# amcpherson/remixt

Measured on AMD Instinct MI355X. Metric: EM iterations/sec (50k seg x 165 states), higher is better.
Workload: dtype f64

## Files before the change

remixt_amd/csrc/rmx_kernels.h:

```cpp
#pragma once
#include "rmx_device.h"
#include "rmx_host.h"
#define SEGL 32
#define SEG_PER_BLOCK (256 / SEGL)
#define TRIAL_SEGL 16
#define RMX_CLUSTER_SPINS (1u << 22)
#define FBK_WKN 128
#define NM_MAX_SAMPLE 1024
#define TRIAL_SEG_PER_BLOCK (256 / TRIAL_SEGL)


__device__ __forceinline__ void state_tables_body(const Dev &d, int cls, int r, const RestartParams &rp) {
    __shared__ unsigned agg_sh;
    if (threadIdx.x == 0) agg_sh = 0u;
    __syncthreads();
    unsigned agg = 0u;
    for (int s = threadIdx.x; s < d.S; s += blockDim.x) {
        const int8_t *cn = d.cn + ((size_t)cls * d.S + s) * d.M * 2;
        const int8_t *tot = d.tot + ((size_t)cls * d.S + s) * d.M;
        double minor = 0., total = 0.;
        for (int m = 0; m < d.M; m++) {
            minor += rp.h[m] * (double)cn[m * 2 + 0];
            total += rp.h[m] * (double)tot[m];
        }
        const unsigned sf = d.sflags[(size_t)cls * d.S + s];
        const bool hdel = sf & 1u, loh = sf & 2u;
        unsigned fl = 0;
        if (!d.nc && hdel) fl |= ST_HDEL_NB;
        double p;
        if (hdel) p = 0.;
        else {
            if (total <= 0.) { fl |= ST_E_TD; p = 0.5; }
            else p = minor / total;
        }
        double M0, M1;
        if (!d.nc && loh) {
            if (p == 0.) p = rp.p[RMX_P_BETABIN_LOH_P];
            else if (p == 1.) p = 1. - rp.p[RMX_P_BETABIN_LOH_P];
            else if (!(fl & ST_E_TD)) fl |= ST_E_LOH;
            M0 = rp.p[RMX_P_BETABIN_LOH_M_0]; M1 = rp.p[RMX_P_BETABIN_LOH_M_1];
            fl |= ST_LOH_M | ST_GZ_ALLELE;
        } else {
            M0 = rp.p[RMX_P_BETABIN_M_0]; M1 = rp.p[RMX_P_BETABIN_M_1];
        }
        if (p <= 0. || (1 - p) <= 0.) fl |= ST_E_BADP;
        const size_t base = ((size_t)r * d.C + cls);
        const size_t si = base * d.SP + s;
        d.stD[si] = total;
        d.stLogD[si] = total > 0. ? log(total) : 0.;
        d.stP[si] = p;
        d.stM[(base * 2 + 0) * d.SP + s] = M0;
        d.stM[(base * 2 + 1) * d.SP + s] = M1;
        const bool ok = !(fl & (ST_E_BADP | ST_E_TD | ST_E_LOH));
        d.stLg[(base * 4 + 0) * d.SP + s] = ok ? lgamma_pos(M0 * p) : 0.;
        d.stLg[(base * 4 + 1) * d.SP + s] = ok ? lgamma_pos(M0 * (1 - p)) : 0.;
        d.stLg[(base * 4 + 2) * d.SP + s] = ok ? lgamma_pos(M1 * p) : 0.;
        d.stLg[(base * 4 + 3) * d.SP + s] = ok ? lgamma_pos(M1 * (1 - p)) : 0.;
        d.stFlags[si] = fl;
        agg |= ((fl & ST_E_TD) ? 1u : 0u) | ((fl & ST_E_LOH) ? 2u : 0u) | (((fl & ST_E_BADP) && !(fl & (ST_E_TD | ST_E_LOH))) ? 4u : 0u);
    }
    if (agg) atomicOr(&agg_sh, agg);
    __syncthreads();
    if (threadIdx.x == 0) d.stFlagsAgg[(size_t)r * d.C + cls] = agg_sh;
}
__global__ void k_state_tables(Dev d, int r0) {
    const int cls = blockIdx.x, r = r0 + blockIdx.y;
    const RestartParams rp = d.rp[r];
    state_tables_body(d, cls, r, rp);
}
__global__ void k_state_tables_one(Dev d, int r, RestartParams rp) {
    if (blockIdx.x == 0 && threadIdx.x == 0) d.rp[r] = rp;
    state_tables_body(d, blockIdx.x, r, rp);
}

__device__ __forceinline__ double seg_const_value(const RestartParams &rp, double x, double y0, double ys, int i) {
    if (i < 4) {
        const double rr = i == 0 ? rp.p[RMX_P_NEGBIN_R_0] : (i == 1 ? rp.p[RMX_P_NEGBIN_HDEL_R_0] : (i == 2 ? rp.p[RMX_P_NEGBIN_R_1] : rp.p[RMX_P_NEGBIN_HDEL_R_1]));
        return lgamma_pos(x + rr) - lgamma_pos(x + 1) - lgamma_pos(rr);
    }
    const double MM = i == 4 ? rp.p[RMX_P_BETABIN_M_0] : (i == 5 ? rp.p[RMX_P_BETABIN_LOH_M_0] : (i == 6 ? rp.p[RMX_P_BETABIN_M_1] : rp.p[RMX_P_BETABIN_LOH_M_1]));
    return (lgamma_pos(ys + 1) - lgamma_pos(y0 + 1) - lgamma_pos(ys - y0 + 1)) - lgamma_pos(ys + MM) + lgamma_pos(MM);
}
__global__ void k_seg_const(Dev d, int r0) {
    const int n = blockIdx.x * blockDim.x + threadIdx.x, r = r0 + blockIdx.y;
    if (n >= d.N) return;
    const RestartParams &rp = d.rp[r];
    const double x = d.x[n], y0 = d.y[2 * (size_t)n], y1 = d.y[2 * (size_t)n + 1], ys = y0 + y1;
    double *sc = d.segc + (size_t)r * 8 * d.N + n;
#pragma unroll
    for (int i = 0; i < 8; i++) sc[(size_t)i * d.N] = seg_const_value(rp, x, y0, ys, i);
}

__global__ void k_framelogprob(Dev d, int r0, int G) {
    const int r = r0 + blockIdx.y;
    const int rows = 256 / G;
    const int n = blockIdx.x * rows + threadIdx.x / G, gl = threadIdx.x % G;
    if (n >= d.N) return;
    const RestartParams &rp = d.rp[r];
    SegCtx sc; load_seg(d, r, n, sc);
    const int cls = d.seg_class[n];
    const double qt0 = d.qt[((size_t)r * d.N + n) * 2], qt1 = d.qt[((size_t)r * d.N + n) * 2 + 1];
    const double qa0 = d.qa[((size_t)r * d.N + n) * 2], qa1 = d.qa[((size_t)r * d.N + n) * 2 + 1];
    const double qs0 = d.qs[((size_t)r * d.N + n) * 2], qs1 = d.qs[((size_t)r * d.N + n) * 2 + 1];
    double *frow = d.f + rs_off(d, r, n);
    unsigned err = 0;
    double vmax = -INFINITY;
    for (int s = gl; s < d.S; s += G) {
        double LT[2], LA[4];
        cell_ll(d, rp, sc, r, cls, s, LT, LA, err);
        double f = 0.;
        f += qt0 * LT[0]; f += qt1 * LT[1];
        f += qa0 * qs0 * LA[0]; f += qa0 * qs1 * LA[1]; f += qa1 * qs0 * LA[2]; f += qa1 * qs1 * LA[3];
        f += cell_prior(d, rp, sc, cls, s);
        if (f != f) err |= RMX_ERR_NAN_F;
        frow[s] = f;
        vmax = f > vmax ? f : vmax;
    }
    vmax = group_max(vmax, G);
    if (gl == 0) d.fmax[(size_t)r * d.N + n] = vmax;
    double *erow = d.fe + rs_off(d, r, n);
    for (int s = gl; s < d.SP; s += G) erow[s] = s < d.S ? exp_fast(frow[s] - vmax) : 0.;
    if (err) atomicOr(&d.err[r], err);
}

#define FB_NBUF 3

struct FbLaunch { int P, NT, BLK, SPAD; };

struct FbArgs {
    int S, SP, M, D, C, N, NBE, cn_max, P, BLK, SPAD, r0, amat_lds, pad_;
    double pen;
    const int32_t *chain_start, *chain_end, *tclass, *brk_slot, *chain_list, *chain_tc, *chain_cls, *be_cls;
    const double *fe, *Wf, *Wb, *pe_lt;
    const int8_t *af, *ab, *tot;
    double *fa, *fb, *mrow;
    uint32_t *err;
    unsigned long long *dbg;
};

typedef const __attribute__((address_space(1))) void *gptr_t;
typedef __attribute__((address_space(3))) void *lptr_t;

#define FB_BARRIER() asm volatile("s_waitcnt lgkmcnt(0)\n\ts_barrier" ::: "memory")

__device__ __forceinline__ void glds16(const void *gsrc, unsigned lds_dst_uniform) {
    unsigned keep;
    asm volatile("s_mov_b32 %0, m0\n\ts_mov_b32 m0, %2\n\ts_nop 0\n\tglobal_load_lds_dwordx4 %1, off\n\ts_mov_b32 m0, %0"
                 : "=&s"(keep) : "v"(gsrc), "s"(lds_dst_uniform) : "memory");
}
__device__ __forceinline__ void glds4(const void *gsrc, unsigned lds_dst_uniform) {
    unsigned keep;
    asm volatile("s_mov_b32 %0, m0\n\ts_mov_b32 m0, %2\n\ts_nop 0\n\tglobal_load_lds_dword %1, off\n\ts_mov_b32 m0, %0"
                 : "=&s"(keep) : "v"(gsrc), "s"(lds_dst_uniform) : "memory");
}
__device__ __forceinline__ void gload8(double &dst, const double *src) {
    asm volatile("global_load_dwordx2 %0, %1, off" : "=v"(dst) : "v"(src) : "memory");
}
__device__ __forceinline__ void gwait8(double &v) { asm volatile("s_waitcnt vmcnt(0)" : "+v"(v) :: "memory"); }
__device__ __forceinline__ void gwait8_after(double &v, double &after) { asm volatile("s_waitcnt vmcnt(0)" : "+v"(v), "+v"(after) :: "memory"); }
__device__ __forceinline__ void gstore8(double *dst, double v) {
    asm volatile("global_store_dwordx2 %0, %1, off\n\ts_nop 1" ::"v"(dst), "v"(v) : "memory");
}
__device__ __forceinline__ unsigned lds_addr(const void *p) { return (unsigned)(size_t)(lptr_t)p; }

#ifdef RMX_FB_STAMPS
#define FB_STAMP(i_) { unsigned long long t_; asm volatile("s_memtime %0\n\ts_waitcnt lgkmcnt(0)" : "=s"(t_) :: "memory"); stamp_acc[i_] += t_ - stamp_last; stamp_last = t_; }
#else
#define FB_STAMP(i_)
#endif
template <int NTMAX>
__global__ __launch_bounds__(NTMAX) void k_fb(FbArgs a) {
    extern __shared__ __align__(16) unsigned char smem_raw[];
    const int chain = a.chain_list[blockIdx.x], r = a.r0 + blockIdx.y, dir = blockIdx.z;
    const int S = a.S, M = a.M, D = a.D, SP = a.SP;
    const int n0 = a.chain_start[chain], n1 = a.chain_end[chain], len = n1 - n0 + 1;
    const int t = threadIdx.x, NT = blockDim.x;
    const int PP = a.P;
    const int p = t / S, o = t - p * S;
    const bool act = p < PP;
    const bool post = t < S;
    const int QPT = (S + PP - 1) / PP;
    const int SPAD = a.SPAD, BLK = a.BLK;
    const int MDP = (M * D + 1) & ~1;
    double *ebuf = (double *)smem_raw;
    double *vec = ebuf + (size_t)FB_NBUF * BLK * SP;
    double *part = vec + 2 * SPAD;
    double *red = part + (size_t)PP * SP;
    double *pel = red + 4;
    double *wa = pel + MDP;
    int *meta = (int *)(wa + 128);
    int8_t *totl = (int8_t *)(meta + FB_NBUF * 2 * 64);
    for (int i = t; i < a.C * S * M; i += NT) totl[i] = a.tot[i];
    for (int i = t; i < 2 * SPAD; i += NT) vec[i] = 0.;
    for (int i = t; i < 128; i += NT) wa[i] = exp(-a.pen * (double)i);
    for (int i = t; i < FB_NBUF * 2 * 64; i += NT) meta[i] = -1;
    unsigned long long *red64 = reinterpret_cast<unsigned long long *>(red);
    if (t < 4) red64[t] = 0ull;

    const size_t rbase = (size_t)r * a.N;
    const double *febase = a.fe + rbase * SP;
    double *outb = (dir == 0 ? a.fa : a.fb) + rbase * SP;
    double *mrow = a.mrow + rbase;
    const double *Wmat = dir == 0 ? a.Wf : a.Wb;

    __syncthreads();

#define ROW(k) (dir == 0 ? n0 + (k) : n1 - (k))
    const int nblk = (len + BLK - 1) / BLK;
    const int elems = BLK * SP / 2;
    const int wave_base = (t >> 6) << 6;
#define FB_ISSUE(b_)                                                                                                   \
    {                                                                                                                  \
        const int slot_ = (b_) % FB_NBUF;                                                                              \
        const int rs_ = dir == 0 ? n0 + (b_) * BLK : n1 - (b_) * BLK - (BLK - 1);                                      \
        for (int i0 = 0; i0 < elems; i0 += NT) {                                                                       \
            const int idx = i0 + t;                                                                                    \
            const int row_ = rs_ + (idx * 2) / SP;                                                                     \
            const unsigned dst_ = __builtin_amdgcn_readfirstlane(lds_addr(ebuf + (size_t)slot_ * BLK * SP + (size_t)(i0 + wave_base) * 2)); \
            if (idx < elems && row_ >= n0 && row_ <= n1) glds16(febase + (size_t)rs_ * SP + (size_t)idx * 2, dst_);   \
        }                                                                                                              \
        if (t < 64) {                                                                                                  \
            const int tn_ = (dir == 0 ? n0 + (b_) * BLK - 1 : n1 - (b_) * BLK - (BLK - 1)) + t;                        \
            const unsigned d0_ = __builtin_amdgcn_readfirstlane(lds_addr(meta + (slot_ * 2 + 0) * 64));                 \
            const unsigned d1_ = __builtin_amdgcn_readfirstlane(lds_addr(meta + (slot_ * 2 + 1) * 64));                 \
            if (t < BLK && tn_ >= n0 && tn_ < n1) { glds4(a.tclass + tn_, d0_); glds4(a.brk_slot + tn_, d1_); }        \
        }                                                                                                              \
    }

    FB_ISSUE(0)
    if (nblk > 1) FB_ISSUE(1)
    asm volatile("s_waitcnt vmcnt(0)" ::: "memory");
    if (nblk > 2) FB_ISSUE(2)
    FB_BARRIER();

    const int rstep = dir == 0 ? SP : -SP;
    double *outp = outb + (size_t)ROW(0) * SP + o;
    double *mptr = mrow + ROW(0);
    const int npw = (S + 63) >> 6;
    {
        double e0 = 0.;
        if (post) { e0 = ebuf[(size_t)(dir == 0 ? 0 : BLK - 1) * SP + o]; vec[o] = e0; gstore8(outp, (dir == 0) ? e0 : 1.0); }
        if ((t >> 6) < npw) {
            const double wm = wave_max_nonneg(e0);
            if ((t & 63) == 0) lds_max_u64(&red64[0], (unsigned long long)__double_as_longlong(wm));
        }
    }
    FB_BARRIER();

    int b = 0, kk = 0, slot = 0;
    int cur = 0, nxt = 1;
    int rc = 0;
    if (a.dbg && t == 0 && blockIdx.x == 0 && blockIdx.y == 0 && blockIdx.z == 0) { a.dbg[0] = clock64(); a.dbg[1] = wall_clock64(); a.dbg[4] = len; }
#ifdef RMX_FB_STAMPS
    unsigned long long stamp_acc[6] = {0, 0, 0, 0, 0, 0}, stamp_last;
    asm volatile("s_memtime %0\n\ts_waitcnt lgkmcnt(0)" : "=s"(stamp_last) :: "memory");
#endif
    for (int k = 1; k < len; k++) {
        FB_STAMP(0)
        if (++kk == BLK) { kk = 0; b++; slot = slot + 1 == FB_NBUF ? 0 : slot + 1; }
        const int kidx = dir == 0 ? kk : BLK - 1 - kk;
        const double *vc = vec + cur * SPAD;
        const int bs = meta[(slot * 2 + 1) * 64 + kidx];
        const int rn = rc + 1 == 3 ? 0 : rc + 1, rz = rn + 1 == 3 ? 0 : rn + 1;
        double inv = 0., e = 0.;
        if ((t >> 6) < npw) {
            double m;
            pow2_scale((unsigned)(red64[rc] >> 32), m, inv);
            if (post) e = ebuf[((size_t)slot * BLK + kidx) * SP + o];
            if (t == 0) { if (dir == 0) gstore8(mptr, m); red64[rz] = 0ull; }
        }
        FB_STAMP(1)
        double acc = 0.;
        if (bs < 0) {
            const double *Wt = Wmat + (size_t)meta[(slot * 2 + 0) * 64 + kidx] * S * S;
            if (act) for (int rr = 0; rr < QPT; rr++) { const int q = p * QPT + rr; if (q < S) acc = fma(vc[q], Wt[(size_t)q * S + o], acc); }
        } else {
            const int tc = meta[(slot * 2 + 0) * 64 + kidx];
            if (t < 64) {
                const unsigned dpe = __builtin_amdgcn_readfirstlane(lds_addr(pel));
                if (t * 2 < MDP) glds16(a.pe_lt + ((size_t)r * a.NBE + bs) * MDP + t * 2, dpe);
            }
            asm volatile("s_waitcnt vmcnt(0)" ::: "memory");
            FB_BARRIER();
            int ca, cb;
            const int8_t *at;
            ca = a.be_cls[2 * bs]; cb = a.be_cls[2 * bs + 1];
            at = (dir == 0 ? a.af : a.ab) + (size_t)tc * S * S;
            const int8_t *tq = totl + (size_t)(dir == 0 ? ca : cb) * S * M;
            const int8_t *to = totl + (size_t)(dir == 0 ? cb : ca) * S * M;
            const int sgn = dir == 0 ? 1 : -1;
            if (act) {
                int to_m[RMX_MAX_CLONES];
#pragma unroll
                for (int c = 0; c < RMX_MAX_CLONES; c++) to_m[c] = c < M ? (int)to[(size_t)o * M + c] : 0;
                for (int rr = 0; rr < QPT; rr++) {
                    const int q = p * QPT + rr;
                    if (q < S) {
                        double wv = wa[(int)at[(size_t)q * S + o]];
#pragma unroll
                        for (int c = 0; c < RMX_MAX_CLONES; c++)
                            if (c < M) { const int dd = sgn * ((int)tq[(size_t)q * M + c] - to_m[c]); wv *= pel[c * D + dd + a.cn_max + 1]; }
                        acc = fma(vc[q], wv, acc);
                    }
                }
            }
        }
        FB_STAMP(2)
        if (act) part[(size_t)p * SP + o] = acc;
        FB_BARRIER();
        FB_STAMP(3)
        outp += rstep;
        if ((t >> 6) < npw) {
// ... 205 lines not shown
        FB_STAMP(0)
        BE_SLOT(k, bs)
        const int cb = (k - 1) & 1, nb = k & 1;
        double e;
        gload8(e, eptr);
        eptr += rstep;
        FB_STAMP(1)
        double acc0[NV], acc1[NV];
#pragma unroll
        for (int v = 0; v < NV; v++) { acc0[v] = 0.; acc1[v] = 0.; }
        FBV_SCALE(cb, ROW(k - 1))
        if (bs < 0) {
            if (act) {
                constexpr int NA = (RPT + 15) / 16;
                double av[NV][NA];
                const double *vb0 = vec + (size_t)cb * SPAD + p * RPT + (lane & 15);
#pragma unroll
                for (int v = 0; v < NV; v++)
#pragma unroll
                    for (int h = 0; h < NA; h++) av[v][h] = vb0[(size_t)v * 2 * SPAD + 16 * h];
                fbv_row_fma<RPT, NV, NA, 0>(av, w0, w1, acc0, acc1);
            }
        } else {
            if (a.code_lds) {
                if (t < (a.PE2P + 1) / 2) {
                    for (int v = 0; v < NVX; v++) {
                        const unsigned dpe = __builtin_amdgcn_readfirstlane(lds_addr(pel + (size_t)(vX + v) * PELW) + (unsigned)(((t >> 6) << 6) * 16));
                        if (vX + v < nv && t * 2 < a.PE2P) glds16(a.pe2_lt + ((size_t)(rg0 + vX + v) * a.NBE + bs) * a.PE2P + t * 2, dpe);
                    }
                }
                if (t < 256) asm volatile("s_waitcnt vmcnt(0)" ::: "memory");
                FB_BARRIER();
                if (act) {
                    constexpr int NA = (RPT + 15) / 16;
                    double av[NVX][NA];
                    const double *vb0 = vec + ((size_t)vX * 2 + cb) * SPAD + p * RPT + (lane & 15);
#pragma unroll
                    for (int v = 0; v < NVX; v++)
#pragma unroll
                        for (int h = 0; h < NA; h++) av[v][h] = vb0[(size_t)v * 2 * SPAD + 16 * h];
                    const unsigned short *crow = codel + (size_t)(p * RPT) * a.SPC + (o0 < a.SPC ? o0 : a.SPC - 2);
                    fbv_row_fma_be<RPT, NVX, NA, 0>(av, crow, a.SPC, wa, pel + (size_t)vX * PELW, PELW, acc0, acc1);
                }
            } else {
                if (t < 64) {
                    for (int v = 0; v < NVX; v++) {
                        const unsigned dpe = __builtin_amdgcn_readfirstlane(lds_addr(pel + (size_t)(vX + v) * MDP));
                        if (vX + v < nv && t * 2 < MDP) glds16(a.pe_lt + ((size_t)(rg0 + vX + v) * a.NBE + bs) * MDP + t * 2, dpe);
                    }
                    asm volatile("s_waitcnt vmcnt(0)" ::: "memory");
                }
                FB_BARRIER();
                const int8_t *at = a.amat_lds ? atl : ((dir == 0 ? a.af : a.ab) + (size_t)tc * S * S);
                if (act) {
                    for (int rr = 0; rr < RPT; rr++) {
                        const int q = p * RPT + rr;
                        if (q >= S) break;
#pragma unroll
                        for (int col = 0; col < 2; col++) {
                            const int o = col == 0 ? o0 : o1;
                            if (o < S) {
                                const double wbase = wa[(int)at[(size_t)q * S + o]];
                                int dd[RMX_MAX_CLONES];
#pragma unroll
                                for (int c = 0; c < RMX_MAX_CLONES; c++) dd[c] = c < M ? sgn * ((int)tcl[(size_t)q * M + c] - (int)tcl[(size_t)o * M + c]) + a.cn_max + 1 : 0;
#pragma unroll
                                for (int v = 0; v < NVX; v++) {
                                    if (vX + v < nv) {
                                        double wv = wbase;
#pragma unroll
                                        for (int c = 0; c < RMX_MAX_CLONES; c++) if (c < M) wv *= pel[(size_t)(vX + v) * MDP + c * D + dd[c]];
                                        const double x = vec[((size_t)(vX + v) * 2 + cb) * SPAD + q];
                                        if (col == 0) acc0[v] = fma(x, wv, acc0[v]); else acc1[v] = fma(x, wv, acc1[v]);
                                    }
                                }
                            }
                        }
                    }
                }
            }
        }
        FB_STAMP(2)
        if (act && o0 < SP) {
#pragma unroll
            for (int v = 0; v < NV; v++) {
                double2 pr; pr.x = acc0[v]; pr.y = acc1[v];
                *reinterpret_cast<double2 *>(part + ((size_t)v * FBV_P + p) * SP + o0) = pr;
            }
        }
        FB_BARRIER();
        FB_STAMP(3)
        outp += rstep;
        unsigned vmax_in = 0u;
        gwait8(e);
        if (post) {
            const double inv = red[pv * 4];
            const double *pp_ = part + (size_t)pv * FBV_P * SP + po;
            const double s0 = pp_[0], s1 = pp_[SP], s2 = pp_[2 * SP], s3 = pp_[3 * SP];
            const double s4 = pp_[4 * SP], s5 = pp_[5 * SP], s6 = pp_[6 * SP], s7 = pp_[7 * SP];
            const double sum = ((((((s0 + s1) + s2) + s3) + s4) + s5) + s6) + s7;
            FB_STAMP(6)
            const double val = sum * inv;
            const double vecv = val * e;
            vec[((size_t)pv * 2 + nb) * SPAD + po] = vecv;
            gstore8(outp, (dir == 0) ? vecv : val);
            vmax_in = (unsigned)__double2hiint(vecv);
        }
        FB_STAMP(7)
        if (postwave) {
            const unsigned wm = wave_max_u32(vmax_in);
            if (lane == 0) lds_max_u32(&red32[(pv * 4 + 2 + nb) * 2], wm);
        }
        FB_STAMP(8)
        FB_BARRIER();
        FB_STAMP(5)
    }
    if (a.dbg && t == 0 && blockIdx.x == 0 && blockIdx.y == 0 && blockIdx.z == 0) { a.dbg[2] = clock64(); a.dbg[3] = wall_clock64(); }
#ifdef RMX_FB_STAMPS
    if (a.dbg && blockIdx.x == 0 && blockIdx.y == 0 && blockIdx.z == 0 && (t == 0 || t == NT - 64)) for (int i = 0; i < 10; i++) a.dbg[8 + (t == 0 ? 0 : 10) + i] = stamp_acc[i];
#endif
    FBV_SCALE((len - 1) & 1, ROW(len - 1))
    if (t < nv) { const double m = red[t * 4 + 1]; if (!(m > 0.) || m == INFINITY) atomicOr(&a.err[rg0 + t], RMX_ERR_NAN_AB); }
#undef FBV_SCALE
#undef ROW
#undef ADJ
#undef BE_SLOT
}

__global__ void k_fill_f64(double *p, size_t n, double v) {
    for (size_t i = (size_t)blockIdx.x * blockDim.x + threadIdx.x; i < n; i += (size_t)gridDim.x * blockDim.x) p[i] = v;
}

struct FbmArgs {
    int S, SP, M, D, C, N, NBE, cn_max, r0, r1, PE2P, SPC, VR, pad_;
    double pen;
    const int32_t *chain_start, *chain_end, *chain_list, *chain_tc, *chain_cls, *be_n, *chain_be;
    const double *fe, *Wf, *Wb, *pe2_lt;
    const int8_t *af, *ab, *tot;
    double *fa, *fb, *mrow;
    uint32_t *err;
    unsigned long long *dbg;
    const int4 *items;
};
__device__ __forceinline__ unsigned row_max_u32(unsigned v) {
    v = max(v, (unsigned)__builtin_amdgcn_update_dpp((int)v, (int)v, 0x121, 0xf, 0xf, false));
    v = max(v, (unsigned)__builtin_amdgcn_update_dpp((int)v, (int)v, 0x122, 0xf, 0xf, false));
    v = max(v, (unsigned)__builtin_amdgcn_update_dpp((int)v, (int)v, 0x124, 0xf, 0xf, false));
    v = max(v, (unsigned)__builtin_amdgcn_update_dpp((int)v, (int)v, 0x128, 0xf, 0xf, false));
    return v;
}
#define FBM_NV 4
#define FBM_DEPTH 4
#define FBM_RING (FBM_DEPTH + 1)
typedef double fbm_d2 __attribute__((ext_vector_type(2)));
template <int OFF> __device__ __forceinline__ void fbm_rd(fbm_d2 &dst, unsigned addr) {
    asm volatile("ds_read_b128 %0, %1 offset:%2" : "=v"(dst) : "v"(addr), "n"(OFF) : "memory");
}
template <int CNT> __device__ __forceinline__ void fbm_wait(fbm_d2 &x) { asm volatile("s_waitcnt lgkmcnt(%1)" : "+v"(x) : "n"(CNT) : "memory"); }
__device__ __forceinline__ int fbm_pos(int q, int i) { return ((((q >> 3) * 4 + (q & 3)) * 4 + i) << 1) + ((q >> 2) & 1); }
template <int PI, int KB> struct fbm_chain {
    static __device__ __forceinline__ void run(fbm_d2 (&ring)[FBM_RING], const double (&w)[KB], unsigned addr, double (&acc)[4]) {
        constexpr int NP = KB / 2;
        constexpr int younger = (NP - 1 - PI) < (FBM_DEPTH - 1) ? (NP - 1 - PI) : (FBM_DEPTH - 1);
        fbm_wait<younger>(ring[PI % FBM_RING]);
        acc[(2 * PI) & 3] = __builtin_amdgcn_mfma_f64_4x4x4f64(ring[PI % FBM_RING].x, w[2 * PI], acc[(2 * PI) & 3], 0, 0, 0);
        acc[(2 * PI + 1) & 3] = __builtin_amdgcn_mfma_f64_4x4x4f64(ring[PI % FBM_RING].y, w[2 * PI + 1], acc[(2 * PI + 1) & 3], 0, 0, 0);
        if constexpr (PI + FBM_DEPTH < NP) fbm_rd<(PI + FBM_DEPTH) * 256>(ring[(PI + FBM_DEPTH) % FBM_RING], addr);
        if constexpr (PI + 1 < NP) fbm_chain<PI + 1, KB>::run(ring, w, addr, acc);
    }
    template <int I> static __device__ __forceinline__ void fill(fbm_d2 (&ring)[FBM_RING], unsigned addr) {
        fbm_rd<I * 256>(ring[I], addr);
        if constexpr (I + 1 < FBM_DEPTH && I + 1 < KB / 2) fill<I + 1>(ring, addr);
    }
};

template <int J> __device__ __forceinline__ void fbm_vfma(double &acc, const double a, const double x) {
    asm("v_fmac_f64_dpp %0, %1, %2 row_newbcast:%3 row_mask:0xf bank_mask:0xf" : "+v"(acc) : "v"(a), "v"(x), "n"(J));
}
#define FBW_G(KB_) (((KB_) + 15) / 16)
template <int KBI, int KB, int NV> struct fbw_chain {
    static __device__ __forceinline__ void run(const double (&av)[NV][FBW_G(KB)], const double (&w)[KB], double (&acc)[NV][2]) {
        fbm_vfma<KBI % 16>(acc[0][KBI & 1], av[0][KBI / 16], w[KBI]);
        if constexpr (NV > 1) fbm_vfma<KBI % 16>(acc[1][KBI & 1], av[1][KBI / 16], w[KBI]);
        if constexpr (KBI + 1 < KB) fbw_chain<KBI + 1, KB, NV>::run(av, w, acc);
    }
};
__device__ __forceinline__ int fbw_pos(int q) { return 64 * (q >> 6) + 16 * (q & 3) + ((q >> 2) & 15); }
template <int P, int KB, int NV> struct fbw_be {
    static __device__ __forceinline__ void run(const double (&av)[NV][FBW_G(KB)], const double (&w)[KB], const unsigned *cw, const int pstride,
                                               const char *tbb, double (&acc)[NV][2]) {
        const unsigned c_ = cw[(size_t)P * pstride];
        const char *r0_ = tbb + (c_ & 0xffffu), *r1_ = tbb + (c_ >> 16);
        double t0[NV], t1[NV];
        if constexpr (NV == 2) {
            const double2 u0_ = *reinterpret_cast<const double2 *>(r0_), u1_ = *reinterpret_cast<const double2 *>(r1_);
            t0[0] = u0_.x; t0[1] = u0_.y; t1[0] = u1_.x; t1[1] = u1_.y;
        } else { t0[0] = *reinterpret_cast<const double *>(r0_); t1[0] = *reinterpret_cast<const double *>(r1_); }
        constexpr int k0 = 2 * P, k1 = 2 * P + 1;
        fbm_vfma<k0 % 16>(acc[0][0], av[0][k0 / 16], w[k0] * t0[0]);
        if constexpr (NV > 1) fbm_vfma<k0 % 16>(acc[1][0], av[1][k0 / 16], w[k0] * t0[1]);
        fbm_vfma<k1 % 16>(acc[0][1], av[0][k1 / 16], w[k1] * t1[0]);
        if constexpr (NV > 1) fbm_vfma<k1 % 16>(acc[1][1], av[1][k1 / 16], w[k1] * t1[1]);
        if constexpr (P + 1 < KB / 2) fbw_be<P + 1, KB, NV>::run(av, w, cw, pstride, tbb, acc);
    }
};

template <int KB, int NV>
__device__ __forceinline__ void fbm_body(const FbmArgs &a, const int chain, const int rg0, const int dir) {
    extern __shared__ __align__(16) unsigned char smem_raw[];
    static_assert(KB % 2 == 0 && KB / 2 >= FBM_DEPTH, "k-blocks come in pairs; ring no deeper than the chain");
    static_assert(NV == 1 || NV == 2 || NV == 4, "restarts per workgroup");
    const int quad = rg0 >> 2, I0 = rg0 & 3;
    const int v_lo = max(a.r0 - rg0, 0), v_hi = min(a.r1 - rg0, NV);
    const int S = a.S, SP = a.SP, M = a.M, D = a.D, VR = a.VR, SPC = a.SPC;
    const int n0 = a.chain_start[chain], n1 = a.chain_end[chain], len = n1 - n0 + 1;
    constexpr int G = FBW_G(KB), VRP = 64 * G;
    const int t = threadIdx.x, NT = blockDim.x, lane = t & 63;
    const int wave = __builtin_amdgcn_readfirstlane(t >> 6), NW = NT >> 6;
    const int kq = lane >> 4, c16 = lane & 15, ib = lane & 3;
    const int id = lane >> 4;
    const bool is_sum = c16 == 15;
    const int col = wave * 15 + c16;
    const double sel0 = ib == 0 ? 1.0 : 0.0, sel1 = ib == 1 ? 1.0 : 0.0;
    (void)sel0; (void)sel1;
    double *vec = (double *)smem_raw;
    double *tab = vec + (size_t)2 * VR * 4;
    double *wa = tab + (size_t)2 * 4 * a.PE2P;
    double *tab2 = wa + 64;
    unsigned *codel = (unsigned *)(tab2 + (size_t)6 * a.PE2P);
    int *bel = (int *)(codel + (size_t)(KB / 2) * 4 * SPC);
    const int be_lo = a.chain_be[2 * chain], be_hi = a.chain_be[2 * chain + 1];
    if (be_hi > be_lo) {
        const int8_t *tg = a.tot + (size_t)a.chain_cls[chain] * S * M;
        const int off_ = a.cn_max + 1, sg_ = dir == 0 ? 1 : -1;
        const unsigned ones_code = (unsigned)(M == 2 ? D : D * D);
        for (int i = t; i < (KB / 2) * 4 * SPC; i += NT) {
            const int ls = i % SPC, pk_ = i / SPC, k_ = pk_ & 3, p_ = pk_ >> 2;
            const int o = (ls >> 4) * 15 + (ls & 15);
            unsigned word = 0;
            for (int h = 0; h < 2; h++) {
                const int q = 4 * (2 * p_ + h) + k_;
                if ((ls & 15) == 15) word |= (ones_code * 48u) << (16 * h);
                else if (q < S && o < S) {
                    int idx = 0;
                    for (int c = 1; c < M; c++) idx = idx * D + sg_ * ((int)tg[q * M + c] - (int)tg[o * M + c]) + off_;
                    word |= ((unsigned)idx * 48u) << (16 * h);
                }
            }
            codel[i] = word;
        }
        for (int i = t; i < be_hi - be_lo; i += NT) bel[i] = a.be_n[be_lo + i];
    }
    for (int i = t; i < 2 * VR * 4; i += NT) vec[i] = 0.;
    for (int i = t; i < 64; i += NT) wa[i] = exp(a.pen * (double)i);
    double w[KB];
    {
        const double *Wmat = (dir == 0 ? a.Wf : a.Wb) + (size_t)a.chain_tc[chain] * S * S;
#pragma unroll
        for (int kb = 0; kb < KB; kb++) {
            const int q = 4 * kb + kq;
            w[kb] = q < S ? (is_sum ? 1.0 : (col < S ? Wmat[(size_t)q * S + col] : 0.)) : 0.;
        }
#pragma unroll
        for (int kb = 0; kb < KB; kb++) asm volatile("" : "+v"(w[kb]));
    }
    __syncthreads();

#define ROW(k) (dir == 0 ? n0 + (k) : n1 - (k))
#define ADJ(k) (dir == 0 ? n0 + (k) - 1 : n1 - (k))
    const int be_step = dir == 0 ? 1 : -1;
    int be_i = dir == 0 ? be_lo : be_hi - 1;
    int be_adj = (be_i >= be_lo && be_i < be_hi) ? __builtin_amdgcn_readfirstlane(bel[be_i - be_lo]) : -2;
    const int rstep = dir == 0 ? SP : -SP;
    const bool mine = !is_sum && (NV == 4 ? col < VR : (col < VRP && id < NV));
    const bool present = id >= v_lo && id < v_hi;
    const bool live = !is_sum && col < S && present;
    const size_t lane_off = ((size_t)(rg0 + (present ? id : v_lo)) * a.N + ROW(0)) * SP + (col < S ? col : S - 1);
    double *outp = (dir == 0 ? a.fa : a.fb) + lane_off;
    const double *eptr = a.fe + lane_off + rstep;
#define FBM_EGET(e_, k_) double e_; gload8(e_, eptr); eptr += rstep;
    const int vbuf = NV == 4 ? VR * 4 : NV * VRP;
    double *vput = vec + (NV == 4 ? fbm_pos(mine ? col : 0, id) : (mine ? id * VRP + fbw_pos(col) : 0));
    const unsigned ap0 = lds_addr(vec + (kq * 4 + ib) * 2);
    const double *avp = vec + 16 * kq + c16;
    const bool scribe = dir == 0 && wave == 0 && is_sum && present;
    double *mptr = a.mrow + (size_t)(rg0 + (present ? id : v_lo)) * a.N + ROW(0);
    if (wave < 4) __builtin_amdgcn_s_setprio(2); else if (wave < 8) __builtin_amdgcn_s_setprio(1); else __builtin_amdgcn_s_setprio(0);
    const int NCH = (a.PE2P * 32 + 1023) >> 10;
#define FBM_FETCH(slot_, buf_)                                                                                                     \
    for (int c_ = wave; c_ < NCH; c_ += NW) {                                                                                      \
        const int e16_ = c_ * 64 + lane;                                                        \
        const unsigned dst_ = __builtin_amdgcn_readfirstlane(lds_addr(tab + (size_t)(buf_) * 4 * a.PE2P) + (unsigned)(c_ * 1024)); \
        if (e16_ * 2 < a.PE2P * 4) glds16(a.pe2_lt + ((size_t)quad * a.NBE + (slot_)) * a.PE2P * 4 + e16_ * 2, dst_);             \
    }
    int be_buf = 0;
    if (be_adj >= 0) FBM_FETCH(be_i, 0)
    {
        double e0 = 0.;
        if (live) { e0 = a.fe[lane_off]; gstore8(outp, (dir == 0) ? e0 : 1.0); }
        if (mine) *vput = live ? e0 : 0.;
    }
    FB_BARRIER();
    if (a.dbg && t == 0 && blockIdx.x == 0) { a.dbg[0] = clock64(); a.dbg[1] = wall_clock64(); a.dbg[4] = len; }
#define FBM_FINISH(sum_, e_, k_)                                                                                                   \
    {                                                                                                                              \
        const unsigned hs_ = (unsigned)__builtin_amdgcn_update_dpp(0, __double2hiint(sum_), 0x15F, 0xf, 0xf, false);    \
        double m_, inv_;                                                                                                           \
        pow2_scale(hs_, m_, inv_);                                                                                                 \
        outp += rstep;                                                                                                             \
        double val_ = (sum_) * inv_;                                                                                               \
        gwait8_after(e_, val_);                                                                 \
        const double vecv_ = val_ * (e_);                                                                                          \
        if (mine) vput[(size_t)((k_) & 1) * vbuf] = live ? vecv_ : 0.;       \
        if (live) gstore8(outp, (dir == 0) ? vecv_ : val_);                                                                        \
        if (scribe) gstore8(mptr, m_);                                           \
        mptr += dir == 0 ? 1 : -1;                                                                                                 \
        PST(1)                                                                                                                     \
        FB_BARRIER();                                                                                                              \
    }
#ifdef RMX_FB_PSTAMPS
    unsigned long long pst_acc[3] = {0, 0, 0}, pst_last;
    asm volatile("s_memtime %0\n\ts_waitcnt lgkmcnt(0)" : "=s"(pst_last) :: "memory");
#define PST(i_) { unsigned long long t_; asm volatile("s_waitcnt lgkmcnt(0)\n\ts_memtime %0\n\ts_waitcnt lgkmcnt(0)" : "=s"(t_) :: "memory"); pst_acc[i_] += t_ - pst_last; pst_last = t_; }
#else
#define PST(i_)
#endif
    int k = 1;
    while (k < len) {
        const int k_be = be_adj >= 0 ? (dir == 0 ? be_adj - n0 + 1 : n1 - be_adj) : len;
        const int k_stop = k_be < len ? k_be : len;
        for (; k < k_stop; k++) {
            PST(2)
            FBM_EGET(e, k)
            double sum;
            if constexpr (NV == 4) {
                fbm_d2 ring[FBM_RING];
                const unsigned apc = ap0 + (unsigned)((k - 1) & 1) * (unsigned)(VR * 32);
                fbm_chain<0, KB>::template fill<0>(ring, apc);
                double acc[4] = {0., 0., 0., 0.};
                fbm_chain<0, KB>::run(ring, w, apc, acc);
                sum = (acc[0] + acc[1]) + (acc[2] + acc[3]);
            } else {
                double av[NV][G], acc[NV][2];
#pragma unroll
                for (int j = 0; j < NV; j++) {
                    acc[j][0] = acc[j][1] = 0.;
#pragma unroll
                    for (int g = 0; g < G; g++) av[j][g] = avp[(size_t)((k - 1) & 1) * vbuf + j * VRP + 64 * g];
                }
                fbw_chain<0, KB, NV>::run(av, w, acc);
                sum = __builtin_amdgcn_mfma_f64_4x4x4f64(sel0, acc[0][0] + acc[0][1], 0., 0, 0, 0);
                if constexpr (NV > 1) sum = __builtin_amdgcn_mfma_f64_4x4x4f64(sel1, acc[1][0] + acc[1][1], sum, 0, 0, 0);
            }
            PST(0)
            FBM_FINISH(sum, e, k)
        }
        if (k < len) {
            const double *tb = tab + (size_t)be_buf * 4 * a.PE2P;
#ifdef RMX_FB_STAMPS
            unsigned long long stamp_acc[6] = {0, 0, 0, 0, 0, 0}, stamp_last;
            asm volatile("s_memtime %0\n\ts_waitcnt lgkmcnt(0)" : "=s"(stamp_last) :: "memory");
#endif
            asm volatile("s_waitcnt vmcnt(0)" ::: "memory");
            FB_BARRIER();
            FB_STAMP(0)
            be_i += be_step;
            be_adj = (be_i >= be_lo && be_i < be_hi) ? __builtin_amdgcn_readfirstlane(bel[be_i - be_lo]) : -2;
            be_buf ^= 1;
            if (be_adj >= 0) FBM_FETCH(be_i, be_buf)
            FB_STAMP(1)
            {
                const double *tw = tab + (size_t)(be_buf ^ 1) * 4 * a.PE2P;
                const int n2_ = M == 2 ? D : D * D, toff_ = a.cn_max + 1;
                for (int e_ = t; e_ <= n2_; e_ += NT) {
                    const int da_ = M == 3 ? abs(e_ / D - toff_) : abs(e_ - toff_), db_ = M == 3 ? abs(e_ % D - toff_) : 0;
                    const int kt_ = a.pad_ == 0 ? da_ + db_ : (da_ != 0) + (db_ != 0);
                    const double f_ = e_ < n2_ ? wa[kt_ & 63] : 1.0;
                    const double2 *row = reinterpret_cast<const double2 *>(tw + (size_t)e_ * 4);
                    double2 r01 = row[0], r23 = row[1];
                    r01.x *= f_; r01.y *= f_; r23.x *= f_; r23.y *= f_;
                    double2 *dst = reinterpret_cast<double2 *>(tab2 + (size_t)e_ * 6);
                    dst[0] = r01; dst[1] = r23;
                }
            }
            FB_BARRIER();
            FBM_EGET(e, k)
            double sum;
            const unsigned *cw = codel + (size_t)kq * SPC + (wave * 16 + c16);
            const char *tbb = reinterpret_cast<const char *>(tab2) + I0 * 8;
            (void)tb;
            if constexpr (NV < 4) {
                double av[NV][G], acc[NV][2];
#pragma unroll
                for (int j = 0; j < NV; j++) {
                    acc[j][0] = acc[j][1] = 0.;
#pragma unroll
                    for (int g = 0; g < G; g++) av[j][g] = avp[(size_t)((k - 1) & 1) * vbuf + j * VRP + 64 * g];
                }
                fbw_be<0, KB, NV>::run(av, w, cw, 4 * SPC, tbb, acc);
                sum = __builtin_amdgcn_mfma_f64_4x4x4f64(sel0, acc[0][0] + acc[0][1], 0., 0, 0, 0);
                if constexpr (NV > 1) sum = __builtin_amdgcn_mfma_f64_4x4x4f64(sel1, acc[1][0] + acc[1][1], sum, 0, 0, 0);
            } else {
            double acc[NV];
#pragma unroll
            for (int j = 0; j < NV; j++) acc[j] = 0.;
            constexpr int NPAIR = KB / 2, CH0 = (NPAIR + 1) / 2;
            unsigned cpk[CH0];
            const fbm_d2 *apd = reinterpret_cast<const fbm_d2 *>(vec + (size_t)((k - 1) & 1) * VR * 4 + (kq * 4 + ib) * 2);
            fbm_d2 an;
            double tn[2][NV];
#define FBM_BE_LOAD(p_, c_)                                                                                                        \
            {                                                                                                                      \
                an = apd[(p_) * 16];                                                                                               \
                const char *r0_ = tbb + ((c_) & 0xffffu), *r1_ = tbb + ((c_) >> 16);                                               \
                if constexpr (NV == 4) {                                                                                           \
                    const double2 u0_ = *reinterpret_cast<const double2 *>(r0_), u1_ = *reinterpret_cast<const double2 *>(r0_ + 16); \
                    const double2 u2_ = *reinterpret_cast<const double2 *>(r1_), u3_ = *reinterpret_cast<const double2 *>(r1_ + 16); \
                    tn[0][0] = u0_.x; tn[0][1] = u0_.y; tn[0][2] = u1_.x; tn[0][3] = u1_.y;                                        \
                    tn[1][0] = u2_.x; tn[1][1] = u2_.y; tn[1][2] = u3_.x; tn[1][3] = u3_.y;                                        \
                } else if constexpr (NV == 2) {                                                                                    \
                    const double2 u0_ = *reinterpret_cast<const double2 *>(r0_), u2_ = *reinterpret_cast<const double2 *>(r1_);    \
                    tn[0][0] = u0_.x; tn[0][1] = u0_.y; tn[1][0] = u2_.x; tn[1][1] = u2_.y;                                        \
                } else {                                                                                                           \
                    tn[0][0] = *reinterpret_cast<const double *>(r0_); tn[1][0] = *reinterpret_cast<const double *>(r1_);          \
                }                                                                                                                  \
            }
#pragma unroll
            for (int c0 = 0; c0 < NPAIR; c0 += CH0) {
#pragma unroll
                for (int u = 0; u < CH0; u++) if (c0 + u < NPAIR) cpk[u] = cw[(size_t)(c0 + u) * 4 * SPC];
                FBM_BE_LOAD(c0, cpk[0])
#pragma unroll
                for (int u = 0; u < CH0; u++) {
                    const int p = c0 + u;
                    if (p >= NPAIR) break;
                    const double ax = an.x, ay = an.y;
                    double t0[NV], t1[NV];
#pragma unroll
                    for (int j = 0; j < NV; j++) { t0[j] = tn[0][j]; t1[j] = tn[1][j]; }
                    if (u + 1 < CH0 && p + 1 < NPAIR) FBM_BE_LOAD(p + 1, cpk[u + 1])
                    const double w0 = w[2 * p], w1 = w[2 * p + 1];
                    double xs[NV], ys[NV];
#pragma unroll
                    for (int j = 0; j < NV; j++) { xs[j] = w0 * t0[j]; ys[j] = w1 * t1[j]; }
                    fbm_vfma<0>(acc[0], ax, xs[0]);
                    if constexpr (NV > 1) fbm_vfma<1>(acc[1], ax, xs[1]);
                    if constexpr (NV > 2) { fbm_vfma<2>(acc[2], ax, xs[2]); fbm_vfma<3>(acc[3], ax, xs[3]); }
                    fbm_vfma<0>(acc[0], ay, ys[0]);
                    if constexpr (NV > 1) fbm_vfma<1>(acc[1], ay, ys[1]);
                    if constexpr (NV > 2) { fbm_vfma<2>(acc[2], ay, ys[2]); fbm_vfma<3>(acc[3], ay, ys[3]); }
                }
            }
#undef FBM_BE_LOAD
#pragma unroll
            for (int j = 0; j < NV; j++) { acc[j] += __shfl_xor(acc[j], 16); acc[j] += __shfl_xor(acc[j], 32); }
            sum = acc[0];
#pragma unroll
            for (int j = 1; j < NV; j++) if (id == j) sum = acc[j];
            }
            FB_STAMP(2)
            FBM_FINISH(sum, e, k)
            FB_STAMP(3)
#ifdef RMX_FB_STAMPS
            if (a.dbg && blockIdx.x == 0 && lane == 0 && (wave & 3) == 0) { for (int i = 0; i < 4; i++) a.dbg[8 + (wave >> 2) * 6 + i] += stamp_acc[i]; if (wave == 0) a.dbg[5] += 1; }
#endif
            k++;
        }
    }
#undef FBM_FINISH
#undef FBM_FETCH
#undef FBM_EGET
#ifdef RMX_FB_PSTAMPS
    if (a.dbg && blockIdx.x == 0 && lane == 0) {
        const int slot = wave == 0 ? 0 : (wave == 4 ? 1 : (wave == 8 ? 2 : (wave == 3 ? 3 : (wave == 7 ? 4 : (wave == NW - 1 ? 5 : -1)))));
        if (slot >= 0) for (int i = 0; i < 3; i++) a.dbg[8 + slot * 3 + i] = pst_acc[i];
    }
#endif
#undef PST
    if (a.dbg && t == 0 && blockIdx.x == 0) { a.dbg[2] = clock64(); a.dbg[3] = wall_clock64(); }
    if (wave == 0) {
        const double *vb = vec + (size_t)((len - 1) & 1) * vbuf;
        double ps = 0.;
        for (int q = c16; q < S; q += 16) ps += vb[NV == 4 ? fbm_pos(q, id) : (id < NV ? id : 0) * VRP + fbw_pos(q)];
        ps = group_sum(ps, 16);
        if (c16 == 0 && present) {
            double m_, inv;
            pow2_scale((unsigned)__double2hiint(ps), m_, inv);
            if (dir == 0) gstore8(a.mrow + (size_t)(rg0 + id) * a.N + ROW(len - 1), m_);
            if (!(m_ > 0.) || m_ == INFINITY) atomicOr(&a.err[rg0 + id], RMX_ERR_NAN_AB);
        }
    }
#undef ROW
#undef ADJ
}
template <int KB>
__global__ __launch_bounds__(768) void k_fbm(FbmArgs a) {
    const int4 it = a.items[blockIdx.x];
    if (it.z == 4) fbm_body<KB, 4>(a, it.x, it.y, it.w);
    else if (it.z == 2) fbm_body<KB, 2>(a, it.x, it.y, it.w);
    else fbm_body<KB, 1>(a, it.x, it.y, it.w);
}

#define FBQ_DEPTH 2
#define FBQ_RING (FBQ_DEPTH + 1)
struct fbq_slot { fbm_d2 a; double b[4]; };
__device__ __forceinline__ void fbq_rd64(double &dst, unsigned addr) { asm volatile("ds_read_b64 %0, %1" : "=v"(dst) : "v"(addr) : "memory"); }
template <int CNT> __device__ __forceinline__ void fbq_wait(fbq_slot &x) {
    asm volatile("s_waitcnt lgkmcnt(%5)" : "+v"(x.a), "+v"(x.b[0]), "+v"(x.b[1]), "+v"(x.b[2]), "+v"(x.b[3]) : "n"(CNT) : "memory");
}
#define FBQ_ADDR(c_, kb_) (((kb_) & 1) ? ((c_)[(kb_) >> 1] >> 16) : ((c_)[(kb_) >> 1] & 0xffffu))
template <int KB> struct fbq_chain {
    static constexpr int NP = KB / 2, NW32 = KB / 2;
    template <int P> static __device__ __forceinline__ void issue(fbq_slot &s, unsigned apc, unsigned wt, const unsigned (&c0)[NW32], const unsigned (&c1)[NW32]) {
        constexpr int k0 = 2 * P, k1 = 2 * P + 1;
        (void)wt;
        unsigned a0 = FBQ_ADDR(c0, k0), a1 = FBQ_ADDR(c1, k0), a2 = FBQ_ADDR(c0, k1), a3 = FBQ_ADDR(c1, k1);
        asm volatile("" : "+v"(a0), "+v"(a1), "+v"(a2), "+v"(a3));
        __builtin_amdgcn_sched_barrier(0);
        fbm_rd<P * 256>(s.a, apc);
        fbq_rd64(s.b[0], a0);
        fbq_rd64(s.b[1], a1);
        fbq_rd64(s.b[2], a2);
        fbq_rd64(s.b[3], a3);
    }
    template <int P> static __device__ __forceinline__ void run(fbq_slot (&ring)[FBQ_RING], unsigned apc, unsigned wt, const unsigned (&c0)[NW32], const unsigned (&c1)[NW32],
                                                                double (&acc)[4]) {
        constexpr int younger = (NP - 1 - P) < (FBQ_DEPTH - 1) ? (NP - 1 - P) : (FBQ_DEPTH - 1);
        fbq_slot &s = ring[P % FBQ_RING];
        fbq_wait<5 * younger>(s);
        acc[0] = __builtin_amdgcn_mfma_f64_4x4x4f64(s.a.x, s.b[0], acc[0], 0, 0, 0);
        acc[1] = __builtin_amdgcn_mfma_f64_4x4x4f64(s.a.x, s.b[1], acc[1], 0, 0, 0);
        acc[2] = __builtin_amdgcn_mfma_f64_4x4x4f64(s.a.y, s.b[2], acc[2], 0, 0, 0);
        acc[3] = __builtin_amdgcn_mfma_f64_4x4x4f64(s.a.y, s.b[3], acc[3], 0, 0, 0);
        __builtin_amdgcn_sched_barrier(0);
        if constexpr (P + FBQ_DEPTH < NP) issue<P + FBQ_DEPTH>(ring[(P + FBQ_DEPTH) % FBQ_RING], apc, wt, c0, c1);
        if constexpr (P + 1 < NP) run<P + 1>(ring, apc, wt, c0, c1, acc);
    }
    template <int I> static __device__ __forceinline__ void fill(fbq_slot (&ring)[FBQ_RING], unsigned apc, unsigned wt, const unsigned (&c0)[NW32], const unsigned (&c1)[NW32]) {
        issue<I>(ring[I], apc, wt, c0, c1);
        if constexpr (I + 1 < FBQ_DEPTH && I + 1 < NP) fill<I + 1>(ring, apc, wt, c0, c1);
    }
};

#define FBQW_DEPTH 2
#define FBQW_RING (FBQW_DEPTH + 1)
struct fbqw_slot { double b[4]; };
template <int CNT> __device__ __forceinline__ void fbqw_wait(fbqw_slot &x) {
    asm volatile("s_waitcnt lgkmcnt(%4)" : "+v"(x.b[0]), "+v"(x.b[1]), "+v"(x.b[2]), "+v"(x.b[3]) : "n"(CNT) : "memory");
}
template <int KB, int NV> struct fbqw_chain {
    static constexpr int NP = KB / 2;
    template <int P> static __device__ __forceinline__ void issue(fbqw_slot &s, const unsigned (&c0)[KB / 2], const unsigned (&c1)[KB / 2]) {
        constexpr int k0 = 2 * P, k1 = 2 * P + 1;
        unsigned a0 = FBQ_ADDR(c0, k0), a1 = FBQ_ADDR(c1, k0), a2 = FBQ_ADDR(c0, k1), a3 = FBQ_ADDR(c1, k1);
        asm volatile("" : "+v"(a0), "+v"(a1), "+v"(a2), "+v"(a3));
        __builtin_amdgcn_sched_barrier(0);
        fbq_rd64(s.b[0], a0); fbq_rd64(s.b[1], a1); fbq_rd64(s.b[2], a2); fbq_rd64(s.b[3], a3);
    }
    template <int P> static __device__ __forceinline__ void run(fbqw_slot (&ring)[FBQW_RING], const double (&av)[NV][FBW_G(KB)], const unsigned (&c0)[KB / 2],
                                                                const unsigned (&c1)[KB / 2], double (&acc0)[NV][2], double (&acc1)[NV][2]) {
        constexpr int younger = (NP - 1 - P) < (FBQW_DEPTH - 1) ? (NP - 1 - P) : (FBQW_DEPTH - 1);
        constexpr int k0 = 2 * P, k1 = 2 * P + 1;
        fbqw_slot &s = ring[P % FBQW_RING];
        fbqw_wait<4 * younger>(s);
        constexpr int O = NV > 1 ? 0 : 1;
        fbm_vfma<k0 % 16>(acc0[0][0], av[0][k0 / 16], s.b[0]);
        if constexpr (NV > 1) fbm_vfma<k0 % 16>(acc0[1][0], av[1][k0 / 16], s.b[0]);
        fbm_vfma<k0 % 16>(acc1[0][0], av[0][k0 / 16], s.b[1]);
        if constexpr (NV > 1) fbm_vfma<k0 % 16>(acc1[1][0], av[1][k0 / 16], s.b[1]);
        fbm_vfma<k1 % 16>(acc0[0][O], av[0][k1 / 16], s.b[2]);
        if constexpr (NV > 1) fbm_vfma<k1 % 16>(acc0[1][O], av[1][k1 / 16], s.b[2]);
        fbm_vfma<k1 % 16>(acc1[0][O], av[0][k1 / 16], s.b[3]);
        if constexpr (NV > 1) fbm_vfma<k1 % 16>(acc1[1][O], av[1][k1 / 16], s.b[3]);
        asm volatile("" : "+v"(acc0[0][0]), "+v"(acc0[0][O]), "+v"(acc1[0][0]), "+v"(acc1[0][O]));
        if constexpr (NV > 1) asm volatile("" : "+v"(acc0[1][0]), "+v"(acc1[1][0]));
        __builtin_amdgcn_sched_barrier(0);
        if constexpr (P + FBQW_DEPTH < NP) issue<P + FBQW_DEPTH>(ring[(P + FBQW_DEPTH) % FBQW_RING], c0, c1);
        if constexpr (P + 1 < NP) run<P + 1>(ring, av, c0, c1, acc0, acc1);
    }
    template <int I> static __device__ __forceinline__ void fill(fbqw_slot (&ring)[FBQW_RING], const unsigned (&c0)[KB / 2], const unsigned (&c1)[KB / 2]) {
        issue<I>(ring[I], c0, c1);
        if constexpr (I + 1 < FBQW_DEPTH && I + 1 < NP) fill<I + 1>(ring, c0, c1);
    }
};
template <int KBI, int KB, int NV> struct fbqw_be {
    static __device__ __forceinline__ void run(const double (&av)[NV][FBW_G(KB)], const char *wtb, const unsigned (&c0)[KB / 2], const unsigned (&c1)[KB / 2],
                                               const int *uplq, const int umul, const int uoff0, const int uoff1, const char *tbb,
                                               double (&acc0)[NV][2], double (&acc1)[NV][2]) {
        const double w0 = *reinterpret_cast<const double *>(wtb + FBQ_ADDR(c0, KBI)), w1 = *reinterpret_cast<const double *>(wtb + FBQ_ADDR(c1, KBI));
        const int uq = __mul24(uplq[4 * KBI], umul);
        const double *r0 = reinterpret_cast<const double *>(tbb + (uq + uoff0)), *r1 = reinterpret_cast<const double *>(tbb + (uq + uoff1));
        fbm_vfma<KBI % 16>(acc0[0][KBI & 1], av[0][KBI / 16], w0 * r0[0]);
        if constexpr (NV > 1) fbm_vfma<KBI % 16>(acc0[1][KBI & 1], av[1][KBI / 16], w0 * r0[1]);
        fbm_vfma<KBI % 16>(acc1[0][KBI & 1], av[0][KBI / 16], w1 * r1[0]);
        if constexpr (NV > 1) fbm_vfma<KBI % 16>(acc1[1][KBI & 1], av[1][KBI / 16], w1 * r1[1]);
        if constexpr (KBI % 2 == 1) __builtin_amdgcn_sched_barrier(0);
        if constexpr (KBI + 1 < KB) fbqw_be<KBI + 1, KB, NV>::run(av, wtb, c0, c1, uplq, umul, uoff0, uoff1, tbb, acc0, acc1);
    }
};

template <int KB, int NV>
__device__ __forceinline__ void fbq_body(const FbmArgs &a, const double *wk, const uint32_t *cnpack, const uint32_t *totpack, const int chain, const int rg0, const int dir) {
    extern __shared__ __align__(16) unsigned char smem_raw[];
    static_assert(KB % 2 == 0 && KB / 2 >= FBQ_DEPTH, "k-blocks come in pairs; ring no deeper than the chain");
    constexpr int NW32 = KB / 2;
    static_assert(NV == 1 || NV == 2 || NV == 4, "restarts per workgroup");
    constexpr int G = FBW_G(KB), VRP = 64 * G;
    const int quad = rg0 >> 2, I0 = rg0 & 3;
    const int v_lo = max(a.r0 - rg0, 0), v_hi = min(a.r1 - rg0, NV);
    const int S = a.S, SP = a.SP, M = a.M, D = a.D, VR = a.VR;
    const int n0 = a.chain_start[chain], n1 = a.chain_end[chain], len = n1 - n0 + 1;
    const int t = threadIdx.x, NT = blockDim.x, lane = t & 63;
    const int wave = __builtin_amdgcn_readfirstlane(t >> 6), NW = NT >> 6;
    const int kq = lane >> 4, c16 = lane & 15, ib = lane & 3, id = lane >> 4;
    const bool is_sum = c16 == 15;
    const int col0 = (2 * wave) * 15 + c16, col1 = (2 * wave + 1) * 15 + c16;
    const int cls = a.chain_cls[chain];
    double *wtab = (double *)smem_raw;
    double *vec = wtab + 64 * 32;
    double *tab = vec + (size_t)2 * VR * 4;
    int *upl = (int *)(tab + (size_t)2 * 4 * a.PE2P);
    double *wup = (double *)(upl + 4 * KB);
    int *bel = (int *)(wup + 64);
    const int be_lo = a.chain_be[2 * chain], be_hi = a.chain_be[2 * chain + 1];
// ... 3484 lines not shown
```

Baseline: 457.0.

## Prefetch emission rows two steps ahead in forward-backward recurrence

Result: slower. 448.8 (-1.8%).

```diff
diff --git a/remixt_amd/csrc/rmx_kernels.h b/remixt_amd/csrc/rmx_kernels.h
--- a/remixt_amd/csrc/rmx_kernels.h
+++ b/remixt_amd/csrc/rmx_kernels.h
@@ -158,6 +158,11 @@
 }
 __device__ __forceinline__ void gwait8(double &v) { asm volatile("s_waitcnt vmcnt(0)" : "+v"(v) :: "memory"); }
 __device__ __forceinline__ void gwait8_after(double &v, double &after) { asm volatile("s_waitcnt vmcnt(0)" : "+v"(v), "+v"(after) :: "memory"); }
+template <int CNT> __device__ __forceinline__ double gwait8_mul(const double &e, const double val) {
+    double r;
+    asm volatile("s_waitcnt vmcnt(%3)\n\tv_mul_f64 %0, %1, %2" : "=v"(r) : "v"(val), "v"(e), "n"(CNT) : "memory");
+    return r;
+}
 __device__ __forceinline__ void gstore8(double *dst, double v) {
     asm volatile("global_store_dwordx2 %0, %1, off\n\ts_nop 1" ::"v"(dst), "v"(v) : "memory");
 }
@@ -669,6 +674,8 @@
 #define FBM_NV 4
 #define FBM_DEPTH 4
 #define FBM_RING (FBM_DEPTH + 1)
+#define FBM_EDIST 2
+#define FBM_ERING (FBM_EDIST + 1)
 typedef double fbm_d2 __attribute__((ext_vector_type(2)));
 template <int OFF> __device__ __forceinline__ void fbm_rd(fbm_d2 &dst, unsigned addr) {
     asm volatile("ds_read_b128 %0, %1 offset:%2" : "=v"(dst) : "v"(addr), "n"(OFF) : "memory");
@@ -794,8 +801,11 @@
     const bool live = !is_sum && col < S && present;
     const size_t lane_off = ((size_t)(rg0 + (present ? id : v_lo)) * a.N + ROW(0)) * SP + (col < S ? col : S - 1);
     double *outp = (dir == 0 ? a.fa : a.fb) + lane_off;
-    const double *eptr = a.fe + lane_off + rstep;
-#define FBM_EGET(e_, k_) double e_; gload8(e_, eptr); eptr += rstep;
+    const long fe_delta = (long)(reinterpret_cast<const char *>(a.fe) - reinterpret_cast<const char *>(dir == 0 ? a.fa : a.fb));
+    const long rstep8 = (long)rstep * 8;
+#define FBM_EADDR(kk_, kdone_) reinterpret_cast<const double *>(reinterpret_cast<const char *>(outp) + (fe_delta + (long)((kk_) - (kdone_)) * rstep8))
+#define FBM_EGET(e_, k_) double e_; gload8(e_, FBM_EADDR(k_, (k_) - 1));
+    const bool wlive = wave * 15 < S && v_lo < v_hi;
     const int vbuf = NV == 4 ? VR * 4 : NV * VRP;
     double *vput = vec + (NV == 4 ? fbm_pos(mine ? col : 0, id) : (mine ? id * VRP + fbw_pos(col) : 0));
     const unsigned ap0 = lds_addr(vec + (kq * 4 + ib) * 2);
@@ -819,15 +829,14 @@
     }
     FB_BARRIER();
     if (a.dbg && t == 0 && blockIdx.x == 0) { a.dbg[0] = clock64(); a.dbg[1] = wall_clock64(); a.dbg[4] = len; }
-#define FBM_FINISH(sum_, e_, k_)                                                                                                   \
+#define FBM_FINISH(sum_, e_, k_, MUL_)                                                                                             \
     {                                                                                                                              \
         const unsigned hs_ = (unsigned)__builtin_amdgcn_update_dpp(0, __double2hiint(sum_), 0x15F, 0xf, 0xf, false);    \
         double m_, inv_;                                                                                                           \
         pow2_scale(hs_, m_, inv_);                                                                                                 \
         outp += rstep;                                                                                                             \
         double val_ = (sum_) * inv_;                                                                                               \
-        gwait8_after(e_, val_);                                                                 \
-        const double vecv_ = val_ * (e_);                                                                                          \
+        const double vecv_ = MUL_(e_, val_);                                \
         if (mine) vput[(size_t)((k_) & 1) * vbuf] = live ? vecv_ : 0.;       \
         if (live) gstore8(outp, (dir == 0) ? vecv_ : val_);                                                                        \
         if (scribe) gstore8(mptr, m_);                                           \
@@ -842,35 +851,52 @@
 #else
 #define PST(i_)
 #endif
+    double er[FBM_ERING];
     int k = 1;
     while (k < len) {
         const int k_be = be_adj >= 0 ? (dir == 0 ? be_adj - n0 + 1 : n1 - be_adj) : len;
         const int k_stop = k_be < len ? k_be : len;
-        for (; k < k_stop; k++) {
-            PST(2)
-            FBM_EGET(e, k)
-            double sum;
-            if constexpr (NV == 4) {
-                fbm_d2 ring[FBM_RING];
-                const unsigned apc = ap0 + (unsigned)((k - 1) & 1) * (unsigned)(VR * 32);
-                fbm_chain<0, KB>::template fill<0>(ring, apc);
-                double acc[4] = {0., 0., 0., 0.};
-                fbm_chain<0, KB>::run(ring, w, apc, acc);
-                sum = (acc[0] + acc[1]) + (acc[2] + acc[3]);
-            } else {
-                double av[NV][G], acc[NV][2];
-#pragma unroll
-                for (int j = 0; j < NV; j++) {
-                    acc[j][0] = acc[j][1] = 0.;
-#pragma unroll
-                    for (int g = 0; g < G; g++) av[j][g] = avp[(size_t)((k - 1) & 1) * vbuf + j * VRP + 64 * g];
-                }
-                fbw_chain<0, KB, NV>::run(av, w, acc);
-                sum = __builtin_amdgcn_mfma_f64_4x4x4f64(sel0, acc[0][0] + acc[0][1], 0., 0, 0, 0);
-                if constexpr (NV > 1) sum = __builtin_amdgcn_mfma_f64_4x4x4f64(sel1, acc[1][0] + acc[1][1], sum, 0, 0, 0);
-            }
-            PST(0)
-            FBM_FINISH(sum, e, k)
+        if (k < k_stop) {
+            const int k_fill = k;
+#pragma unroll
+            for (int i = 0; i < FBM_EDIST; i++) { const int kk = min(k + i, len - 1); gload8(er[i], FBM_EADDR(kk, k - 1)); }
+            for (;;) {
+#pragma unroll
+                for (int s = 0; s < FBM_ERING; s++) {
+                    PST(2)
+                    { const int kk = min(k + FBM_EDIST, len - 1); gload8(er[(s + FBM_EDIST) % FBM_ERING], FBM_EADDR(kk, k - 1)); }
+                    const bool steady = wlive && k - k_fill >= FBM_EDIST;
+#define FBM_MUL_PLAIN(e_, v_) (steady ? gwait8_mul<2 * FBM_EDIST>(e_, v_) : gwait8_mul<FBM_EDIST>(e_, v_))
+                    double sum;
+                    if constexpr (NV == 4) {
+                        fbm_d2 ring[FBM_RING];
+                        const unsigned apc = ap0 + (unsigned)((k - 1) & 1) * (unsigned)(VR * 32);
+                        fbm_chain<0, KB>::template fill<0>(ring, apc);
+                        double acc[4] = {0., 0., 0., 0.};
+                        fbm_chain<0, KB>::run(ring, w, apc, acc);
+                        sum = (acc[0] + acc[1]) + (acc[2] + acc[3]);
+                    } else {
+                        double av[NV][G], acc[NV][2];
+#pragma unroll
+                        for (int j = 0; j < NV; j++) {
+                            acc[j][0] = acc[j][1] = 0.;
+#pragma unroll
+                            for (int g = 0; g < G; g++) av[j][g] = avp[(size_t)((k - 1) & 1) * vbuf + j * VRP + 64 * g];
+                        }
+                        fbw_chain<0, KB, NV>::run(av, w, acc);
+                        sum = __builtin_amdgcn_mfma_f64_4x4x4f64(sel0, acc[0][0] + acc[0][1], 0., 0, 0, 0);
+                        if constexpr (NV > 1) sum = __builtin_amdgcn_mfma_f64_4x4x4f64(sel1, acc[1][0] + acc[1][1], sum, 0, 0, 0);
+                    }
+                    PST(0)
+                    FBM_FINISH(sum, er[s], k, FBM_MUL_PLAIN)
+#undef FBM_MUL_PLAIN
+                    if (++k >= k_stop) goto plain_run_done;
+                }
+            }
+plain_run_done:
+            static_assert(FBM_ERING == 3, "the drain names the ring's registers");
+            if (wlive) asm volatile("s_waitcnt vmcnt(1)" : "+v"(er[0]), "+v"(er[1]), "+v"(er[2]) :: "memory");
+            else asm volatile("s_waitcnt vmcnt(0)" : "+v"(er[0]), "+v"(er[1]), "+v"(er[2]) :: "memory");
         }
         if (k < len) {
             const double *tb = tab + (size_t)be_buf * 4 * a.PE2P;
@@ -976,7 +1002,9 @@
             for (int j = 1; j < NV; j++) if (id == j) sum = acc[j];
             }
             FB_STAMP(2)
-            FBM_FINISH(sum, e, k)
+#define FBM_MUL_BE(e_, v_) (gwait8_after(e_, v_), (v_) * (e_))
+            FBM_FINISH(sum, e, k, FBM_MUL_BE)
+#undef FBM_MUL_BE
             FB_STAMP(3)
 #ifdef RMX_FB_STAMPS
             if (a.dbg && blockIdx.x == 0 && lane == 0 && (wave & 3) == 0) { for (int i = 0; i < 4; i++) a.dbg[8 + (wave >> 2) * 6 + i] += stamp_acc[i]; if (wave == 0) a.dbg[5] += 1; }
@@ -987,6 +1015,7 @@
 #undef FBM_FINISH
 #undef FBM_FETCH
 #undef FBM_EGET
+#undef FBM_EADDR
 #ifdef RMX_FB_PSTAMPS
     if (a.dbg && blockIdx.x == 0 && lane == 0) {
         const int slot = wave == 0 ? 0 : (wave == 4 ? 1 : (wave == 8 ? 2 : (wave == 3 ? 3 : (wave == 7 ? 4 : (wave == NW - 1 ? 5 : -1)))));
```
